# utiasSTARS/pyslam

Measured on AMD Instinct MI355X. Metric: ms/LM-iter (Jac build + J^T J + Schur solve), stereo BA @ 500k residuals, lower is better.
Workload: dtype f64

## Files before the change

### include/pyslam_hip.h

```cpp
#ifndef PYSLAM_HIP_H
#define PYSLAM_HIP_H

#include <stdint.h>

#ifdef __cplusplus
extern "C" {
#endif

typedef struct ps_problem ps_problem;

typedef struct ps_problem_desc {
    int32_t dof;
    int32_t num_poses;
    const double*  poses;
    const int32_t* pose_rid;
    int32_t num_points;
    const double*  points;
    const int32_t* point_vid;

    int64_t num_obs;
    const int32_t* obs_pose;
    const int32_t* obs_point;
    const double*  obs_uvd;
    const int32_t* obs_grp;
// ... 140 lines not shown
int ps_covariance_column(ps_problem* h, int kind, int index, int comp, double tol, int max_iters,
                         int* iters_out, double* relres_out);

#define PS_COV_DENSE_MAX_UNKNOWNS 12288
int ps_covariance_marginals(ps_problem* h, double* pose_blocks ,
                            double* point_blocks );
int ps_covariance_pose_blocks(ps_problem* h, int64_t n, const int32_t* a, const int32_t* b,
                              double* out );
int ps_covariance_cross_blocks(ps_problem* h, int64_t n, const int32_t* kind_a, const int32_t* a,
                               const int32_t* kind_b, const int32_t* b, double* out );

int ps_triangulate(ps_problem* h, int64_t n, const int32_t* vids , int refine_iters, double min_parallax_deg,
                   int write_back, double* points_out , int32_t* status_out );

int ps_get_reduced_system(ps_problem* h, int32_t* row_ptr, int32_t* col_idx,
                          double* vals, double* g);
int ps_get_landmark_factors(ps_problem* h, double* cinv , double* c );
int ps_debug_reproj_blocks(ps_problem* h, double* r , double* jpose ,
                           double* jpoint );
int ps_debug_factor_blocks(ps_problem* h, double* r, double* j1, double* j2);
int ps_debug_table_checksums(ps_problem* h, uint64_t* out, int capacity, int* count);

int ps_set_option(ps_problem* h, const char* name, double value);

int ps_set_profiling(ps_problem* h, int enabled);
int ps_get_stage_times(ps_problem* h, double* ms , int64_t* counts, int reset);

int ps_dense_normal_solve(const double* J, const double* r, int32_t m, int32_t n,
                          double* dx, double* covariance );

int ps_sparse_normal_solve(int32_t m, int32_t n, const int32_t* j_row_ptr, const int32_t* j_col, const double* j_val,
                           const int32_t* jt_row_ptr, const int32_t* jt_col, const double* jt_val,
                           const double* r, const double* rhs, double tol, int32_t max_iters,
                           double* dx, int32_t* iters_out, double* relres_out);

int ps_sparse_normal_direct(int32_t m, int32_t n, const int32_t* j_row_ptr, const int32_t* j_col, const double* j_val,
                            const int32_t* jt_row_ptr, const int32_t* jt_col, const double* jt_val,
                            const double* r, const double* rhs, int32_t refine_steps, double* dx, double* relres_out);

int ps_debug_band_inverse(const double* a, int32_t ncb, int32_t dof, int32_t bw, int32_t chunk_nodes, float* ainv_out,
                          double* elapsed_us);
int ps_debug_factor_stress(const double* a, int32_t ncb, int32_t dof, int32_t bw, int32_t mode, int32_t launches, int32_t lowprio,
                           int32_t aggressor, int32_t* n_diff, int32_t* n_pivot);

int ps_ransac_transforms(const double* pts_1, const double* pts_2, int32_t batch, int32_t n, double* T_out);
int ps_ransac_cost(const double* T, int32_t num_hyp, const double* pts_1, const double* obs_2, int32_t num_pts,
// ... 81 lines not shown
```

### pyslam_amd/_native.py

```python
import ctypes as C
import os

import numpy as np

_HERE = os.path.dirname(os.path.abspath(__file__))
LIB_PATH = os.path.join(_HERE, 'lib', 'libpyslam_hip.so')
if os.environ.get('PYSLAM_AMD_MEASURE') == '1':
    LIB_PATH = os.path.join(_HERE, 'lib', 'libpyslam_hip_measure.so')

c_i32p = C.POINTER(C.c_int32)
c_f64p = C.POINTER(C.c_double)
c_u8p = C.POINTER(C.c_uint8)
PS_NUM_STAGES = 12
STAGE_NAMES = ['landmark_pass', 'pose_pass', 'schur_pairs', 'pose_factors', 'pcg',
               'backsub', 'update', 'cost', 'iteration_total', 'cg_kernel', 'allreduce', 'pack_unpack']


class ProblemDesc(C.Structure):
    _fields_ = [
        ('dof', C.c_int32), ('num_poses', C.c_int32), ('poses', c_f64p), ('pose_rid', c_i32p),
        ('num_points', C.c_int32), ('points', c_f64p), ('point_vid', c_i32p),
        ('num_obs', C.c_int64), ('obs_pose', c_i32p), ('obs_point', c_i32p), ('obs_uvd', c_f64p),
        ('obs_grp', c_i32p),
        ('num_cams', C.c_int32), ('cams', c_f64p), ('num_stiff3', C.c_int32), ('stiff3', c_f64p),
# ... 89 lines not shown
    'ps_solve_lm': (C.c_int, [H, C.POINTER(LmOptions), C.c_double, C.c_int, c_f64p, C.c_int32, C.POINTER(C.c_int32),
                              C.POINTER(C.c_int32), C.POINTER(C.c_double), c_i32p, c_f64p, c_f64p, c_f64p]),
    'ps_gn_finish': (C.c_int, [H, C.c_int, c_f64p, c_f64p, c_f64p]),
    'ps_gn_solve_finish': (C.c_int, [H, C.c_double, C.c_int, C.c_int, c_f64p, c_f64p, c_f64p,
                                     C.POINTER(C.c_int), c_f64p]),
    'ps_set_collective': (C.c_int, [H, C.c_void_p, C.c_void_p]),
    'ps_set_segment_exchange': (C.c_int, [H, C.c_void_p, C.c_int32, C.c_int32, C.c_int64, C.c_int64, C.POINTER(C.c_int64), C.c_int64,
                                         C.POINTER(C.c_int64), C.POINTER(C.c_int64), C.POINTER(C.c_int64)]),
    'ps_shard_buffer': (C.c_int, [H, C.POINTER(C.c_void_p)]),
    'ps_gn_solve_finish_enqueue': (C.c_int, [H, C.c_double, C.c_int, C.c_int, C.c_int]),
    'ps_gn_result': (C.c_int, [H, C.POINTER(C.c_int), c_f64p, c_f64p, C.POINTER(C.c_int), c_f64p]),
    'ps_covariance_begin': (C.c_int, [H]),
    'ps_covariance_column': (C.c_int, [H, C.c_int, C.c_int, C.c_int, C.c_double, C.c_int, C.POINTER(C.c_int), c_f64p]),
    'ps_covariance_marginals': (C.c_int, [H, c_f64p, c_f64p]),
    'ps_covariance_pose_blocks': (C.c_int, [H, C.c_int64, c_i32p, c_i32p, c_f64p]),
    'ps_covariance_cross_blocks': (C.c_int, [H, C.c_int64, c_i32p, c_i32p, c_i32p, c_i32p, c_f64p]),
    'ps_triangulate': (C.c_int, [H, C.c_int64, c_i32p, C.c_int, C.c_double, C.c_int, c_f64p, c_i32p]),
    'ps_get_reduced_system': (C.c_int, [H, c_i32p, c_i32p, c_f64p, c_f64p]),
    'ps_get_landmark_factors': (C.c_int, [H, c_f64p, c_f64p]),
    'ps_debug_reproj_blocks': (C.c_int, [H, c_f64p, c_f64p, c_f64p]),
    'ps_debug_factor_blocks': (C.c_int, [H, c_f64p, c_f64p, c_f64p]),
    'ps_debug_table_checksums': (C.c_int, [H, C.POINTER(C.c_uint64), C.c_int, C.POINTER(C.c_int)]),
    'ps_set_option': (C.c_int, [H, C.c_char_p, C.c_double]),
    'ps_set_profiling': (C.c_int, [H, C.c_int]),
    'ps_get_stage_times': (C.c_int, [H, c_f64p, C.POINTER(C.c_int64), C.c_int]),
    'ps_ransac_transforms': (C.c_int, [c_f64p, c_f64p, C.c_int32, C.c_int32, c_f64p]),
    'ps_ransac_cost': (C.c_int, [c_f64p, C.c_int32, c_f64p, c_f64p, C.c_int32, c_f64p, C.c_double, c_u8p, c_i32p]),
    'ps_ransac_frame_to_frame': (C.c_int, [c_f64p, c_f64p, c_f64p, C.c_int32, c_i32p, C.c_int32, C.c_int32, c_f64p,
                                           C.c_double, c_f64p, c_i32p, c_i32p, c_i32p, c_f64p, c_u8p]),
    'ps_twoview_hypotheses': (C.c_int, [c_f64p, c_f64p, C.c_int32, c_i32p, C.c_int32, c_f64p, C.c_double, c_f64p, c_i32p, c_u8p]),
    'ps_twoview_score': (C.c_int, [c_f64p, C.c_int32, c_f64p, c_f64p, C.c_int32, c_f64p, C.c_double, c_u8p, c_i32p]),
    'ps_twoview_ransac': (C.c_int, [c_f64p, c_f64p, C.c_int32, c_i32p, C.c_int32, c_f64p, C.c_double, C.c_int32, c_f64p, c_f64p,
                                    c_u8p, c_i32p, c_f64p]),
    'ps_photometric_create': (C.c_int, [C.POINTER(PhotoDesc), C.c_void_p, C.POINTER(H)]),
    'ps_photometric_destroy': (C.c_int, [H]),
    'ps_photometric_set_pose': (C.c_int, [H, c_f64p]),
    'ps_photometric_get_pose': (C.c_int, [H, c_f64p]),
    'ps_photometric_eval_cost': (C.c_int, [H, c_f64p, C.POINTER(C.c_int64)]),
    'ps_photometric_normal_equations': (C.c_int, [H, c_f64p, c_f64p, c_f64p, C.POINTER(C.c_int64)]),
    'ps_photometric_iteration': (C.c_int, [H, C.c_int32, C.c_int32, c_f64p, c_f64p]),
    'ps_dense_create': (C.c_int, [C.c_int32, C.c_int32, C.c_int32, C.c_int32, C.c_void_p, C.POINTER(H)]),
    'ps_dense_destroy': (C.c_int, [H]),
    'ps_dense_upload': (C.c_int, [H, C.c_int32, C.c_int32, C.c_int32, C.c_int32, C.c_void_p, c_f64p]),
    'ps_dense_make_tables': (C.c_int, [H, C.c_int32, C.c_int32, c_i32p, c_f64p, C.c_double, C.c_double, C.c_double]),
    'ps_dense_track': (C.c_int, [H, C.c_int32, C.c_int32, C.c_int32, c_i32p, c_i32p, C.POINTER(SolveOptions), C.c_int32,
                                 C.c_double, c_f64p, c_f64p, c_i32p, c_f64p, C.c_int32]),
# ... 118 lines not shown
```

### pyslam_amd/csrc/ps_abi_problem.h

```cpp


const char* ps_last_error(void) { return g_err.c_str(); }

int ps_device_count(void) {
    int n = 0;
    if (hipGetDeviceCount(&n) != hipSuccess) return 0;
    return n;
}

int ps_warm_up(void) {
    static std::once_flag once;
    static int rc = 0;
    std::call_once(once, [] {
        void* p = nullptr;
        if (hipMalloc(&p, 256) != hipSuccess) { rc = fail("hipMalloc failed (no usable HIP device?)"); return; }
        hipLaunchKernelGGL(k_zero4, dim3(1), dim3(256), 0, 0, (size_t)8, (double*)p, (size_t)0, (double*)nullptr, (size_t)0,
                           (double*)nullptr, (size_t)0, (double*)nullptr);
        double hostw[4] = {0, 0, 0, 0};
        (void)hipMemsetAsync(p, 0, 256, 0);
        (void)hipMemcpyAsync((char*)p + 128, p, 64, hipMemcpyDeviceToDevice, 0);
        (void)hipMemcpyAsync(hostw, p, sizeof(hostw), hipMemcpyDeviceToHost, 0);
        if (hipDeviceSynchronize() != hipSuccess) rc = fail("the warm-up launch failed");
        hipFree(p);
        hipFuncAttributes a;
// ... 699 lines not shown
            if (rb >= 0) { cs.push_back({diag_slot[rb], base + 2 * DD, 0}); gl[rb].push_back(base + 3 * DD + D); }
            if (ra >= 0 && rb >= 0) {
                if (ra == rb) return fail("pose-pose edge connects a pose with itself");
                cs.push_back({slot_of(ra, rb), base + DD, 0});
                cs.push_back({slot_of(rb, ra), base + DD, 1});
            }
        }
        std::stable_sort(cs.begin(), cs.end(), [](const C& x, const C& y) { return x.slot < y.slot; });
        std::vector<int32_t> eslots, eptr, ediag, gptr(nr + 1, 0), gitems;
        std::vector<int2> eitems(cs.size());
        for (size_t k = 0; k < cs.size(); ++k) {
            eitems[k] = make_int2(cs[k].off, cs[k].tr);
            if (k == 0 || cs[k].slot != cs[k - 1].slot) { eslots.push_back(cs[k].slot); eptr.push_back((int32_t)k); }
        }
        eptr.push_back((int32_t)cs.size());
        for (int32_t s : eslots) {
            const int row = (int)(std::upper_bound(row_ptr.begin(), row_ptr.end(), s) - row_ptr.begin()) - 1;
            ediag.push_back(col_idx[s] == row ? 1 : 0);
        }
        for (int r = 0; r < nr; ++r) { gptr[r + 1] = gptr[r] + (int32_t)gl[r].size(); gitems.insert(gitems.end(), gl[r].begin(), gl[r].end()); }
        h->nes = (int)eslots.size();
        if (h->upload(&h->eslots, eslots) || h->upload(&h->eptr, eptr) || h->upload(&h->eslot_diag, ediag) ||
            h->upload(&h->eitems, eitems) || h->upload(&h->gptr, gptr) || h->upload(&h->gitems, gitems)) return -1;
    }

    lap("factor lists");
    const size_t nvec = (size_t)nr * D;
    h->npartA = std::max(1, nr);
    h->npartB = std::max(1, cdiv(nr, D == 6 ? PS_PCG_BR(6) : PS_PCG_BR(3)));
    h->hist_cap = 4098;
    if (h->alloc(&h->x, nvec) || h->alloc(&h->r, nvec) || h->alloc(&h->z, nvec) || h->alloc(&h->p0, nvec) ||
        h->alloc(&h->p1, nvec) || h->alloc(&h->q, nvec) || h->alloc(&h->Minv, (size_t)nr * DD) ||
        h->alloc(&h->rz_part, h->npartB) || h->alloc(&h->rr_part, h->npartB) || h->alloc(&h->pq_part, h->npartA) ||
        h->alloc(&h->hist, 2 * (size_t)h->hist_cap)) return -1;
    {
        std::vector<int32_t> brow_of(nnzb), ident(nnzb);
        for (int r = 0; r < nr; ++r) for (int b = row_ptr[r]; b < row_ptr[r + 1]; ++b) brow_of[b] = r;
        for (int b = 0; b < nnzb; ++b) ident[b] = b;
        if (h->upload(&h->brow_of, brow_of) || h->upload(&h->ident_slot, ident)) return -1;
        if (h->alloc(&h->Linv, (size_t)nr * DD)) return -1;
    }
    if (h->zero(h->x, nvec * sizeof(double)) || h->zero(h->p0, nvec * sizeof(double)) || h->zero(h->p1, nvec * sizeof(double))) return -1;

    lap("pcg workspace");
    h->ncost_obs = N > 0 ? std::min(2048, cdiv(N, 256)) : 0;
    h->ncost_fac = F > 0 ? std::min(1024, cdiv(F, 256)) : 0;
// ... 42 lines not shown
    char* whost = (char*)h->words_host;
    h->h_scalars = (double*)(whost + 0);      h->h_scalars_dev = (double*)(wdev + 0);
    h->h_status = (int32_t*)(whost + 256);    h->h_status_dev = (int32_t*)(wdev + 256);
    h->h_seq = (long long*)(whost + 512);     h->h_seq_dev = (long long*)(wdev + 512);
    h->h_shard = (double*)(whost + 768);      h->h_shard_dev = (double*)(wdev + 768);
    h->h_setup = (long long*)(whost + 1024);  h->h_setup_dev = (long long*)(wdev + 1024);
    h->h_ldi_fro = (double*)(whost + 1280);   h->h_ldi_fro_dev = (double*)(wdev + 1280);
    h->h_early = (long long*)(whost + 1536);  h->h_early_dev = (long long*)(wdev + 1536);
    h->h_lmfail = (long long*)(whost + 1792); h->h_lmfail_dev = (long long*)(wdev + 1792);
    h->h_mo_hist = (double*)(whost + 2048);   h->h_mo_hist_dev = (double*)(wdev + 2048);
    if (h->alloc(&h->arrivals, 2)) return -1;
    if (h->zero(h->arrivals, 2 * sizeof(int32_t))) return -1;
    if (h->arena_close()) return -1;
    HIP_OK(hipStreamSynchronize(h->stream));
    if (nr >= 16 && nr * D > h->direct_max && h->pcg_variant == 1 && !ps_env("PS_LAZY_COARSE")) {
        if (build_coarse(h)) return -1;
        HIP_OK(hipStreamSynchronize(h->stream));
        lap("two-level structures");
    }
    if (ldi_eligible(h) && h->ldi_direct_ok && h->N == 0 && h->F > 0 && !h->ldi_stream &&
        !ps_pool().take(ps_pool().side_streams, &h->ldi_stream))
        HIP_OK(hipStreamCreateWithFlags(&h->ldi_stream, hipStreamNonBlocking));
    lap("scalars + final sync");
    guard.ok = true;
    *out = h;
    return 0;
}

int ps_problem_create(const ps_problem_desc* d_in, void* stream, ps_problem** out) {
    return problem_create(d_in, nullptr, stream, out);
}

int ps_problem_create_hybrid(const ps_problem_desc* d_in, const ps_host_rows_desc* rows, void* stream, ps_problem** out) {
    if (!rows) return fail("null argument");
    return problem_create(d_in, rows, stream, out);
}

int ps_set_host_rows(ps_problem* h, const double* rows, int64_t num, double cost) {
    if (!h) return fail("null argument");
    if (!h->hybrid) return fail("ps_set_host_rows: the handle has no host rows (ps_problem_create_hybrid)");
    if (num != h->FH) return fail("ps_set_host_rows: row count differs from the create call's");
    if (num > 0 && !rows) return fail("null argument");
    const size_t FROW = 3 * (size_t)h->D * h->D + 2 * (size_t)h->D;
    if (num > 0) {
        HIP_OK(hipMemcpyAsync(h->fscratch + (size_t)h->F * FROW, rows, (size_t)num * FROW * sizeof(double), hipMemcpyHostToDevice, h->stream));
        HIP_OK(hipStreamSynchronize(h->stream));
// ... 7 lines not shown
```

### pyslam_amd/csrc/ps_abi_solver.h

```cpp

int ps_get_info(ps_problem* h, ps_problem_info* info) {
    if (!h || !info) return fail("null argument");
    info->dof = h->D; info->num_poses = h->P; info->num_reduced = h->nr; info->num_points = h->L;
    info->num_var_points = h->nv; info->num_obs = h->N; info->num_edges = h->F; info->num_priors = 0;
    info->reduced_nnzb = h->nnzb; info->num_pairs = h->npairs;
    info->reduce_count = ((long)h->nnzb + h->nr) / 2 * h->D * h->D + (long)h->nr * h->D + 3;
    info->device_bytes = (int64_t)h->dev_bytes;
    info->cg_restarts = h->cg_fallbacks;
    info->cg_kernel_launches = h->cg_kernel_launches;
    info->ldi_solves = h->ldi_solves; info->ldi_fallbacks = h->ldi_fallbacks; info->ldi_seeds = h->ldi_seeds;
    info->xcg_fused_solves = h->xf_solves; info->xcg_fused_fallbacks = h->xf_fallbacks;
    info->cg_persist_solves = h->cp_launches; info->cg_persist_failures = h->cp_failures;
    info->cg_persist_refused = h->cp_refused; info->persist_cus = h->persist_cus;
    info->persist_cus_needed = h->cp_ok ? h->cp_cus_needed : (h->xp_ok ? h->xp_cus_needed : 0);
    info->landmark_passes_taken_over = h->prelm_used;
    return 0;
}

int ps_eval_cost(ps_problem* h, int include_all_constant, double* cost) {
    if (!h || !cost) return fail("null argument");
    if (include_all_constant && h->fuse_cost == 1 && lm_cost_possible(h)) { if (lm_cost_pass(h, h->lin_lambda, SC_COST)) return -1; }
    else if (cost_pass(h, include_all_constant, SC_COST)) return -1;
    if (read_scalars(h)) return -1;
    *cost = h->h_scalars[SC_COST];
// ... 5 lines not shown
    if (!h) return fail("null argument");
    h->last_cost = h->prev_cost = -1.0;
    return linearize(h, lambda);
}

static int ensure_shard_pack(ps_problem* h) {
    if (h->shard_pack) return 0;
    const int nr = h->nr, DD = h->D * h->D;
    std::vector<int32_t> up, upT;
    for (int r = 0; r < nr; ++r)
        for (int b = h->h_row_ptr[r]; b < h->h_row_ptr[r + 1]; ++b) {
            const int c = h->h_col_idx[b];
            if (c < r) continue;
            up.push_back(b);
            const int32_t* lo = h->h_col_idx.data() + h->h_row_ptr[c];
            const int32_t* hi = h->h_col_idx.data() + h->h_row_ptr[c + 1];
            const int32_t* it = std::lower_bound(lo, hi, r);
            if (it == hi || *it != r) return fail("reduced block pattern is not symmetric");
            upT.push_back((int32_t)(it - h->h_col_idx.data()));
        }
    h->nup = (long)up.size();
    h->pack_count = h->nup * DD + (long)nr * h->D + 2 + 1;
    if (h->upload(&h->up_slot, up) || h->upload(&h->upT_slot, upT) || h->alloc(&h->shard_pack, (size_t)h->pack_count)) return -1;
    return 0;
}

int ps_reduce_buffer(ps_problem* h, void** dev_ptr, int64_t* count) {
    if (!h || !dev_ptr || !count) return fail("null argument");
    if (ensure_shard_pack(h)) return -1;
    *dev_ptr = h->shard_pack; *count = h->pack_count;
    return 0;
}

int ps_shard_pack(ps_problem* h) {
    if (!h) return fail("null argument");
    if (ensure_shard_pack(h)) return -1;
    const long ntail = (long)h->nr * h->D + 2;
    const int nb = (int)std::min<long>(4096, cdiv(h->pack_count, 256));
    if (h->D == 6) hipLaunchKernelGGL(k_shard_pack<6>, dim3(nb), dim3(256), 0, h->stream, h->nup, h->up_slot, h->S, ntail, h->g, h->status, h->shard_pack);
    else hipLaunchKernelGGL(k_shard_pack<3>, dim3(nb), dim3(256), 0, h->stream, h->nup, h->up_slot, h->S, ntail, h->g, h->status, h->shard_pack);
    return 0;
}

int ps_shard_unpack(ps_problem* h) {
    if (!h) return fail("null argument");
    h->prelin_valid = h->prelm_valid = false;
// ... 199 lines not shown
    {
        StageTimer tpk(h, PS_ST_PACK);
        if (h->D == 6) hipLaunchKernelGGL(k_seg_pack<6>, dim3(nb1), dim3(256), 0, h->stream, h->nup, h->up_slot, h->S, ntail, h->g, h->status, T, h->seg_nmine, h->seg_mine, h->seg_in, h->seg_maxlen);
        else hipLaunchKernelGGL(k_seg_pack<3>, dim3(nb1), dim3(256), 0, h->stream, h->nup, h->up_slot, h->S, ntail, h->g, h->status, T, h->seg_nmine, h->seg_mine, h->seg_in, h->seg_maxlen);
    }
    {
        StageTimer tar(h, PS_ST_ALLREDUCE);
        if (h->seg_allgather(h->seg_in, h->seg_all, (size_t)h->seg_maxlen, NCCL_F64, h->nccl_comm, h->stream))
            return fail("ncclAllGather of the reduced system's segments failed");
    }
    {
        StageTimer tpk(h, PS_ST_PACK);
        if (h->D == 6) hipLaunchKernelGGL(k_seg_sum<6>, dim3(nb2), dim3(256), 0, h->stream, h->seg_ndst, h->seg_dst, h->seg_src_ptr, h->seg_src_off, h->seg_all, T, h->seg_world, h->seg_maxlen, h->nup, h->up_slot, h->upT_slot, h->S, ntail, h->g, h->status);
        else hipLaunchKernelGGL(k_seg_sum<3>, dim3(nb2), dim3(256), 0, h->stream, h->seg_ndst, h->seg_dst, h->seg_src_ptr, h->seg_src_off, h->seg_all, T, h->seg_world, h->seg_maxlen, h->nup, h->up_slot, h->upT_slot, h->S, ntail, h->g, h->status);
    }
    return 0;
}

int ps_set_collective(ps_problem* h, void* nccl_all_reduce_fn, void* nccl_comm) {
    if (!h) return fail("null argument");
    if (h->hybrid && nccl_comm) return fail("a hybrid handle (host rows) is not landmark-sharded");
    h->nccl_allreduce = (ps_problem::allreduce_fn)nccl_all_reduce_fn;
    h->nccl_comm = nccl_comm;
    return 0;
}

int ps_shard_buffer(ps_problem* h, void** dev_ptr) {
    if (!h || !dev_ptr) return fail("null argument");
    *dev_ptr = h->shard_buf;
    return 0;
}

int ps_gn_solve_finish_enqueue(ps_problem* h, double pcg_tol, int pcg_max_iters, int linesearch, int first) {
    if (!h) return fail("null argument");
    if (h->nr == 0 || h->pcg_variant != 1) return fail("ps_gn_solve_finish_enqueue needs the fused CG and a reduced system");
    pcg_tol = resolve_pcg_tol(h, pcg_tol);
    if (first && z_of_last_linearize(h, "ps_gn_solve_finish_enqueue")) return -1;
    h->shard_out = true;
    h->no_repeat = !(h->nccl_allreduce && h->nccl_comm);
    struct Reset { ps_problem* h; ~Reset() { h->shard_out = false; h->no_repeat = false; } } reset{h};
    if (first) {
        HIP_OK(hipMemsetAsync(h->scalars + SC_DXP2, 0, sizeof(double), h->stream));
        if (!h->coarse_built && build_coarse(h)) return -1;
        if (!(h->nccl_allreduce && h->nccl_comm) && h->xf_skip == 0) h->xf_skip = 1;
        if (h->cg_explicit) { if (h->D == 6 ? xcg_setup<6>(h, pcg_max_iters, true) : xcg_setup<3>(h, pcg_max_iters, true)) return -1; }
        else if (h->D == 6 ? cg_fused_setup<6>(h, pcg_max_iters, true) : cg_fused_setup<3>(h, pcg_max_iters, true)) return -1;
// ... 547 lines not shown
    else if (n == "ldi_cap") { if (value < 1 || value > 64) return fail("ldi_cap out of range (1 .. 64)"); h->ldi_cap = (int)value; }
    else if (n == "ldi_cost_tol") { if (!(value >= 0)) return fail("ldi_cost_tol must be >= 0"); h->ldi_cost_tol = value; }
    else if (n == "ldi_refresh_its") { if (value < 0 || value > 64) return fail("ldi_refresh_its out of range (0 .. 64)"); h->ldi_refresh_its = (int)value; }
    else if (n == "ldi_direct") { h->ldi_direct_ok = value != 0.0; h->ldi_direct = value > 0.0; }
    else if (n == "direct_fused") h->direct_fused = value != 0.0;
    else if (n == "ldi_seed_lag") { if (value < 1 || value > 16) return fail("ldi_seed_lag out of range (1 .. 16)"); h->ldi_seed_lag = (int)value; }
    else if (n == "ldi_seed_steps") { if (value < 1 || value > 40) return fail("ldi_seed_steps out of range (1 .. 40)"); h->ldi_seed_steps = (int)value; }
    else if (n == "coarse_refresh_every") { if (value < 1 || value > 16) return fail("coarse_refresh_every must be 1..16"); h->xcg_refresh_every = (int)value; }
    else if (n == "coarse_lag_x") { h->lagx = value != 0.0; h->lci_next = -1; h->side_todo = false; }
    else if (n == "cg_lds") h->cg_lds = value != 0.0;
    else if (n == "cg_persist") h->cg_persist = value != 0.0;
    else if (n == "xcg_persist") h->xcg_persist = value != 0.0;
    else if (n == "cg_persist_spin") { if (value < 0 || value > 1e7) return fail("cg_persist_spin out of range"); h->cp_spin = (unsigned)value; }
    else if (n == "cg_explicit") { h->explicit_ok = value != 0.0; h->coarse_built = false; }
    else if (n == "big_chol") h->big_chol = value != 0.0;
    else if (n == "fused_motion_only") h->mo_fused = value != 0.0;
    else if (n == "direct_max_unknowns") { if (value < 0 || value > 90) return fail("direct_max_unknowns must be 0..90"); h->direct_max = (int)value; }
    else if (n == "coarse_basis") { h->coarse_basis = value != 0.0; h->lci_next = -1; h->side_todo = false; }
    else if (n == "profile_every") { if (value < 1) return fail("profile_every must be >= 1"); h->prof_every = (int)value; }
    else if (n == "cg_margin") { if (value < 0 || value > 64) return fail("cg_margin out of range"); h->cg_margin = (int)value; }
    else if (n == "cg_split_min_rows") { h->cg_split_min_rows = (int)value; h->coarse_built = false; }
    else if (n == "cg_explicit_min_rows") { h->cg_explicit_min_rows = (int)value; h->coarse_built = false; }
    else if (n == "pcg_chunk") { if (value < 1 || value > 4096) return fail("pcg_chunk out of range"); h->pcg_chunk = (int)value; }
    else return fail("unknown option: " + n);
    return 0;
}

int ps_reset_solver_state(ps_problem* h) {
    if (!h) return fail("null argument");
    h->prelin_valid = h->prelm_valid = false;
    if (!h->solver_touched) {
        h->last_cost = h->prev_cost = h->snap_cost = -1.0;
        h->solve_horizon = -1;
        return 0;
    }
    h->solver_touched = false;
    HIP_OK(hipStreamSynchronize(h->stream));
    if (h->side) HIP_OK(hipStreamSynchronize(h->side));
    if (h->ldi_stream) HIP_OK(hipStreamSynchronize(h->ldi_stream));
    drain_timers(h);
    h->lci_next = -1; h->lci_cur = 0;
    h->side_todo = false; h->side_ready = false; h->side_pending = false; h->acdone_pending = false;
    h->xcg_side_todo = false; h->xcg_lag_count = 0; h->xcg_held = 0;
    h->xcg_its_ref = 0; h->xcg_good_held = 0; h->xcg_ref_pending = false;
    h->xcg_tag[0] = h->xcg_tag[1] = -1.0; h->xcg_tag_lambda[0] = h->xcg_tag_lambda[1] = 0.0;
    h->xcg_setup_cost = -1.0; h->xcg_setup_lambda = 0.0;
    h->mc_active = false; h->last_setup_lagx = false; h->xf_skip = 0;
// ... 67 lines not shown
```

### pyslam_amd/csrc/ps_core.hip

```cpp
#include <hip/hip_runtime.h>

#include <algorithm>
#include <array>
#include <map>
#include <atomic>
#include <chrono>
#include <thread>
#include <climits>
#include <cmath>
#include <cstdio>
#include <cstring>
#include <memory>
#include <mutex>
#include <string>
#include <vector>

#include "pyslam_hip.h"
#include "ps_kernels.h"
#include "ps_ransac.h"
#include "ps_k_twoview.h"
#include "ps_photo.h"
#include "ps_k_dense.h"
#include "ps_k_feat.h"
#include "ps_sparse.h"
// ... 135 lines not shown
    LObs* pobs = nullptr;
    PItem* pitems = nullptr;
    int npitems = 0;
    int32_t* pitem_ptr = nullptr;
    double* ppartial = nullptr;
    int2* pairs = nullptr;
    int npair_items = 0, pair_per_xcd = 0;
    PairItem* pair_xitems = nullptr;
    int schur_tiles = 1, ncomb = 0;
    bool has_diag_tasks = false;
    double* Spart = nullptr;
    PairItem* comb_items = nullptr;
    int32_t* comb_tasks = nullptr;
    FactorGroup* fgroups = nullptr;
    int32_t *f_i = nullptr, *f_j = nullptr, *f_grp = nullptr;
    double *f_Tinv = nullptr, *fscratch = nullptr;
    int32_t *eslots = nullptr, *eptr = nullptr, *eslot_diag = nullptr, *gptr = nullptr, *gitems = nullptr;
    int2* eitems = nullptr;
    int nes = 0;
    int32_t *row_ptr = nullptr, *col_idx = nullptr, *diag_slot = nullptr;
    double* red = nullptr;
    long red_count = 0;
    double *S = nullptr, *g = nullptr, *red_cost = nullptr;
    std::vector<int32_t> h_row_ptr, h_col_idx;
    std::vector<int32_t> h_vid_of_slot;
    double *x = nullptr, *r = nullptr, *z = nullptr, *p0 = nullptr, *p1 = nullptr, *q = nullptr, *Minv = nullptr;
    double *rz_part = nullptr, *rr_part = nullptr, *pq_part = nullptr, *hist = nullptr;
    int npartA = 0, npartB = 0, hist_cap = 0, last_pcg_iters = 0;
    int pcg_variant = 1;
    int pcg_chunk = 8;
    double *Linv = nullptr, *cg_r[2] = {}, *cg_w[2] = {}, *cg_s[2] = {}, *cg_gd[2] = {}, *cg_xh = nullptr;
    int32_t* brow_of = nullptr;
    double* cg_p = nullptr;
    double* Saug = nullptr;
    int32_t* ident_slot = nullptr;
    int coarse_req = -1;
    int G = 0, ncb = 0, nc = 0, nr_aug = 0, nnzb_aug = 0;
    size_t cg_cap = 0, saug_cap = 0;
    int32_t *pnode = nullptr, *slo = nullptr, *shi = nullptr, *run_lo = nullptr, *run_hi = nullptr,
            *arow_ptr = nullptr, *acol_idx = nullptr, *aug_slot = nullptr, *fine_nnz = nullptr;
    double *pw0 = nullptr, *pw1 = nullptr, *SZ = nullptr, *Ac = nullptr, *tvec = nullptr, *chol_scratch = nullptr;
    int coarse_basis = 1;
    double *Bmat = nullptr, *bgv = nullptr, *SB = nullptr, *BSZ = nullptr;
    double *Bmat2[2] = {}, *X2[2] = {}, *Mpart = nullptr;
    bool lagx_ok = false;
    int lagx = 1;
// ... 318 lines not shown
    int arena_close() {
        arena_open = false;
        if (arena_poisoned) arena_used = PS_ARENA_BYTES;
        if (arena_used) HIP_OK(hipMemcpyAsync(arena_dev, arena_host, arena_used, hipMemcpyHostToDevice, stream));
        return 0;
    }
    void arena_release() {
        PsPool& pool = ps_pool();
        if (arena_dev && !pool.give(pool.dev_arenas, (void*)arena_dev)) hipFree(arena_dev);
        if (arena_host && !pool.give(pool.host_arenas, (void*)arena_host)) hipHostFree(arena_host);
        if (words_host && !pool.give(pool.host_words, words_host)) hipHostFree(words_host);
        arena_dev = arena_host = nullptr; words_host = nullptr;
    }
};

inline void cov_release(ps_problem* h) {
    if (!h->cov_buf) return;
    hipStreamSynchronize(h->stream);
    hipFree(h->cov_buf);
    h->cov_buf = nullptr;
    h->cov_sigma_epoch = -1;
}

#include "ps_host_cg.h"
#include "ps_host_ldi.h"
#include "ps_host_iteration.h"
#include "ps_host_build.h"

extern "C" {

#include "ps_abi_problem.h"
#include "ps_abi_solver.h"
#include "ps_abi_cov.h"
#include "ps_abi_triang.h"
#include "ps_abi_small.h"
#include "ps_abi_twoview.h"
#include "ps_abi_dense.h"
#include "ps_abi_feat.h"

}
```

### pyslam_amd/csrc/ps_host_cg.h

```cpp

namespace {

struct StageTimer {
    ps_problem* h;
    int stage;
    hipEvent_t a = nullptr, b = nullptr;
    int slot = -1;
    StageTimer(ps_problem* h_, int st, int level = 2) : h(h_), stage(st) {
        if (h->profiling < level) return;
        if (h->profiling == 1 && h->prof_every > 1 &&
            h->prof_tick % h->prof_every != (st == PS_ST_CG_KERNEL ? h->prof_every / 2 : 0)) return;
        if (h->ev_used + 2 > h->ev_pool.size()) {
            for (int i = 0; i < 64; ++i) { hipEvent_t e; hipEventCreate(&e); h->ev_pool.push_back(e); }
        }
        slot = (int)h->ev_used;
        a = h->ev_pool[h->ev_used++];
        b = h->ev_pool[h->ev_used++];
        hipEventRecord(a, h->stream);
    }
    void stop() {
        if (!a) return;
        hipEventRecord(b, h->stream);
        h->pending.push_back({stage, slot});
        a = nullptr;
// ... 848 lines not shown
    if (iters_out) *iters_out = total_its;
    if (relres_out) *relres_out = rel * reduced;
    h->last_pcg_iters = total_its;
    return rc;
}

int linearize(ps_problem* h, double lambda, bool allow_prelm) {
    h->solver_touched = true;
    h->prelin_valid = false;
    const bool lm_done = allow_prelm && h->prelm_valid && h->prelm_lambda == lambda && h->nv > 0;
    h->prelm_valid = false;
    h->lin_lmfail_tag = lm_done ? h->prelm_tag : 0;
    if (lm_done) ++h->prelm_used;
    h->lin_lambda = lambda;
    h->params_moved_since_lin = false; h->z_foreign = false;
    ++h->prof_tick;
    h->cov_ready = false;
    cov_release(h);
    h->status_clean = false;
    if (h->ldi_sread_pending) {
        HIP_OK(hipStreamWaitEvent(h->stream, h->ev_ldi_sread, 0));
        h->ldi_sread_pending = false;
    }
    HIP_OK(hipMemsetAsync(h->red, 0, h->red_count * sizeof(double) + ST_NWORDS * sizeof(int32_t), h->stream));
    if (h->nv > 0 && !lm_done) {
        StageTimer t(h, PS_ST_LANDMARK);
        const ObsWide wl{h->sidx_l, h->stiff_tab};
#define PS_LM_LAUNCH(W) hipLaunchKernelGGL(k_landmark_pass<W>, dim3(cdiv(h->nv, 256 / PS_LM_GROUP)), dim3(256), 0, h->stream, h->nv, h->lm_ptr, \
                           h->lm_point, h->lobs, h->poses, h->points, h->pose_rid, h->ogroups, lambda, h->Z,                       \
                           h->Cinv, h->cvec, h->status, h->lm_ablate, wl)
#define PS_LMP_LAUNCH(W) hipLaunchKernelGGL((k_landmark_pass_packed<W, false>), dim3(cdiv(h->lmw_nwaves, 4)), dim3(256), 0, h->stream, h->lmw_nwaves, \
                           h->lmw_first, h->lm_ptr, h->lm_point, h->lobs, h->poses, h->points, h->pose_rid, h->ogroups, lambda, h->Z,      \
                           h->Cinv, h->cvec, h->status, wl, (const int32_t*)nullptr, (double*)nullptr, (long long*)nullptr, 0LL)
        if (h->lm_packed && h->lmw_nwaves > 0 && !h->lm_ablate) { if (h->wide_obs) PS_LMP_LAUNCH(true); else PS_LMP_LAUNCH(false); }
        else if (h->wide_obs) PS_LM_LAUNCH(true); else PS_LM_LAUNCH(false);
#undef PS_LMP_LAUNCH
#undef PS_LM_LAUNCH
    }
    bool fin_in_combine = false, fin_in_pairs = false;
    static const bool schur_split_env = ps_env("PS_SCHUR_SPLIT") != nullptr;
    if (h->npitems > 0) {
        StageTimer t(h, PS_ST_POSE);
        const ObsWide wp{h->sidx_p, h->stiff_tab};
        const int per_xcd = h->pose_xcd ? cdiv(h->npitems, 8) : 0;
        const int nblk = per_xcd ? 8 * per_xcd : h->npitems;
        if (h->wide_obs)
            hipLaunchKernelGGL(k_pose_pass<true>, dim3(nblk), dim3(256), 0, h->stream, h->pitems, h->pobs,
                               h->poses, h->points, h->ogroups, h->Cinv, h->cvec, h->ppartial, lambda != 0.0 ? 1 : 0, wp, h->npitems, per_xcd);
        else
            hipLaunchKernelGGL(k_pose_pass<false>, dim3(nblk), dim3(256), 0, h->stream, h->pitems, h->pobs,
                               h->poses, h->points, h->ogroups, h->Cinv, h->cvec, h->ppartial, lambda != 0.0 ? 1 : 0, wp, h->npitems, per_xcd);
        fin_in_combine = h->Spart && h->npair_items > 0 && !h->has_diag_tasks && h->D == 6;
        fin_in_pairs = !h->Spart && h->schur_pipeline && h->npair_items > 0 && !h->has_diag_tasks && h->D == 6 && !schur_split_env;
        if (!fin_in_combine && !fin_in_pairs)
            hipLaunchKernelGGL(k_pose_finalize, dim3(h->nr), dim3(64), 0, h->stream, h->nr, h->pitem_ptr,
                               h->ppartial, h->diag_slot, lambda, h->S, h->g);
    }
    if (h->npair_items > 0) {
        StageTimer t(h, PS_ST_SCHUR, 1);
        const bool split2 = schur_split_env;
        const int halfp = split2 ? (h->pair_per_xcd / 2 + 3) / 4 * 4 : h->pair_per_xcd;
        static const int lds_pad = ps_env("PS_SCHUR_LDS_PAD") ? atoi(ps_env("PS_SCHUR_LDS_PAD")) : 0;
        auto launch_pairs = [&](int nblk, int lds, int from, int to) {
            if (!h->schur_pipeline)
                hipLaunchKernelGGL(k_schur_pairs, dim3(nblk), dim3(256), lds, h->stream, h->pair_per_xcd, h->pair_xitems, h->pairs,
                                   h->Z, h->S, h->Spart, h->schur_ablate, from, to);
            else {
#ifdef PS_MEASURE
                auto k = h->schur_ablate == 0 ? k_schur_pairs_db<0> : h->schur_ablate == 1 ? k_schur_pairs_db<1> :
                         h->schur_ablate == 2 ? k_schur_pairs_db<2> : h->schur_ablate == 3 ? k_schur_pairs_db<3> :
                         h->schur_ablate == 4 ? k_schur_pairs_db<4> : k_schur_pairs_db<5>;
#else
                auto k = k_schur_pairs_db<0>;
#endif
// ... 219 lines not shown
```

### pyslam_amd/csrc/ps_k_linearize.h

```cpp
#pragma once

#define PS_LM_GROUP 16

PS_DEV double group16_sum(double v) {
    v = dpp_shift_add<0x111, 0xf, 0xf>(v);
    v = dpp_shift_add<0x112, 0xf, 0xf>(v);
    v = dpp_shift_add<0x114, 0xf, 0xe>(v);
    v = dpp_shift_add<0x118, 0xf, 0xc>(v);
    return __shfl(v, (int)(threadIdx.x & 63) | 15, 64);
}

#define PS_ZROW 16

PS_DEV void lm_emit_m(const ReprojEval& ev, double M00, double M10, double M11, double M20, double M21,
                      double M22, double* __restrict__ m) {
#pragma unroll
    for (int a = 0; a < 3; ++a) {
        const double w0 = ev.Jp[a] * ev.Jl[0] + ev.Jp[6 + a] * ev.Jl[3] + ev.Jp[12 + a] * ev.Jl[6];
        const double w1 = ev.Jp[a] * ev.Jl[1] + ev.Jp[6 + a] * ev.Jl[4] + ev.Jp[12 + a] * ev.Jl[7];
        const double w2 = ev.Jp[a] * ev.Jl[2] + ev.Jp[6 + a] * ev.Jl[5] + ev.Jp[12 + a] * ev.Jl[8];
        m[3 * a] = w0 * M00;
        m[3 * a + 1] = w0 * M10 + w1 * M11;
        m[3 * a + 2] = w0 * M20 + w1 * M21 + w2 * M22;
    }
// ... 152 lines not shown
    acc[17] += y * F[2][2] - z * F[1][2];
    acc[18] += z * F[0][1] - x * F[2][1];
    acc[19] += z * F[0][2] - x * F[2][2];
    acc[20] += x * F[1][2] - y * F[0][2];
}

#define PS_NPOSE_ACC 33
#ifndef PS_POSE_TRANSPOSE
#define PS_POSE_TRANSPOSE 1
#endif
typedef const __attribute__((address_space(1))) void* ps_gptr_t;
typedef __attribute__((address_space(3))) void* ps_lptr_t;

#ifndef PS_POSE_WAVES
#define PS_POSE_WAVES 3
#endif
template <bool WIDE>
__global__ __launch_bounds__(256) __attribute__((amdgpu_waves_per_eu(PS_POSE_WAVES, 8))) void k_pose_pass(
    const PItem* __restrict__ items,
    const LObs* __restrict__ pobs ,
    const double* __restrict__ poses, const double* __restrict__ points,
    const ObsGroup* __restrict__ groups, const double* __restrict__ Cinv,
    const double* __restrict__ cvec, double* __restrict__ partial, int want_diag ,
    ObsWide wide, int nitems, int per_xcd )
{
    __shared__ double red[4][PS_NPOSE_ACC];
#if PS_POSE_TRANSPOSE
    __shared__ double tr[4][64 * 17];
#endif
    const int item = per_xcd > 0 ? (int)(blockIdx.x & 7) * per_xcd + (int)(blockIdx.x >> 3) : (int)blockIdx.x;
    if (item >= nitems) return;
    const PItem it = items[item];
    const int w = threadIdx.x >> 6, lane = threadIdx.x & 63;
    const Se3 T = se3_load(poses + 12 * (size_t)it.pad);
    double acc[PS_NPOSE_ACC];
#pragma unroll
    for (int k = 0; k < PS_NPOSE_ACC; ++k) acc[k] = 0.0;
    for (int i = it.start + threadIdx.x; i < it.end; i += 256) {
        const LObs o = pobs[i];
        const int v = PS_POSE_OF(o) - 1;
        const double pw[3] = {points[3 * (size_t)o.point], points[3 * (size_t)o.point + 1], points[3 * (size_t)o.point + 2]};
        double m[6] = {0, 0, 0, 0, 0, 0}, c0 = 0.0, c1 = 0.0, c2 = 0.0;
        if (v >= 0) {
            const double* ci = Cinv + 6 * (size_t)v;
#pragma unroll
            for (int k = 0; k < 6; ++k) m[k] = ci[k];
            c0 = cvec[3 * (size_t)v]; c1 = cvec[3 * (size_t)v + 1]; c2 = cvec[3 * (size_t)v + 2];
        }
        ReprojEval ev;
        reproj_eval_obs<true, true, WIDE>(T, pw, &o.u, groups, PS_GRP_OF(o), wide, i, ev);
        double G[6], t3[3];
        {
// ... 355 lines not shown
```

### pyslam_amd/device.py

```python
import ctypes as C

import numpy as np

from pyslam_amd import _native as nat


COVARIANCE_MARGINALS_LIMIT = 12288


def _solve_options(o, opt, linesearch=None):
    o.max_iters, o.allow_nondecreasing_steps = int(opt.max_iters), int(bool(opt.allow_nondecreasing_steps))
    o.max_nondecreasing_steps = int(opt.max_nondecreasing_steps)
    o.linesearch = int(bool(opt.linesearch_max_iters > 0 if linesearch is None else linesearch))
    o.min_update_norm, o.min_cost = float(opt.min_update_norm), float(opt.min_cost)
    o.min_cost_decrease, o.lm_lambda = float(opt.min_cost_decrease), float(getattr(opt, 'lm_lambda', 0.))
    return o


class DeviceProblem:
    def __init__(self, lp, stream=None, extra_pairs=None):
        lib = nat.require_gpu()
        self._lib = lib
        self.lp = lp
        self.dof = lp.dof
# ... 363 lines not shown
    def get_info(self):
        info = nat.ProblemInfo()
        nat.check(self._lib.ps_get_info(self._h, C.byref(info)))
        return {k: getattr(info, k) for k, _ in nat.ProblemInfo._fields_}

    def cg_restarts(self):
        info = nat.ProblemInfo()
        nat.check(self._lib.ps_get_info(self._h, C.byref(info)))
        return int(info.cg_restarts)

    def cg_kernel_launches(self):
        info = nat.ProblemInfo()
        nat.check(self._lib.ps_get_info(self._h, C.byref(info)))
        return int(info.cg_kernel_launches)

    def cg_persist_counts(self):
        info = nat.ProblemInfo()
        nat.check(self._lib.ps_get_info(self._h, C.byref(info)))
        return int(info.cg_persist_solves), int(info.cg_persist_failures)

    def set_option(self, name, value):
        nat.check(self._lib.ps_set_option(self._h, name.encode(), float(value)))

    def set_profiling(self, level=2):
        nat.check(self._lib.ps_set_profiling(self._h, int(level)))

    def stage_times(self, reset=False):
        ms = (C.c_double * nat.PS_NUM_STAGES)()
        cnt = (C.c_int64 * nat.PS_NUM_STAGES)()
        nat.check(self._lib.ps_get_stage_times(self._h, ms, cnt, int(reset)))
        return {n: (ms[i], cnt[i]) for i, n in enumerate(nat.STAGE_NAMES)}


def dense_normal_solve(J, r, want_covariance=False):
    lib = nat.require_gpu()
    J = np.ascontiguousarray(J, dtype=np.float64)
    r = np.ascontiguousarray(r, dtype=np.float64).reshape(-1)
    m, n = J.shape
    dx = np.zeros(n)
    cov = np.zeros((n, n)) if want_covariance else None
    nat.check(lib.ps_dense_normal_solve(nat.f64p(J), nat.f64p(r), m, n, nat.f64p(dx), nat.f64p(cov)))
    return (dx, cov) if want_covariance else dx


def band_inverse(A, ncb, dof, bw, chunk_nodes=0):
    lib = nat.require_gpu()
# ... 267 lines not shown
```

Before: 0.3064.

## Replace full reduction-buffer memset with targeted slot zeroing fused into pose pass

Instead of memsetting the whole Schur/gradient reduction buffer every linearization, a host-side analysis finds the block slots that are not fully overwritten by a single writer. Extra blocks are appended to the pose-pass kernel launch to zero only those slots plus the gradient/status tail. This removes a large memset pass over S each iteration and folds the remaining clearing into an existing launch. It relies on the single-writer analysis being correct, is gated off for sharded, extra-pair or non-pipelined configurations, and adds a get_option read-back API.

Result: faster. 0.3031 (median of 6 runs) (-1.1%).

```diff
diff --git a/include/pyslam_hip.h b/include/pyslam_hip.h
--- a/include/pyslam_hip.h
+++ b/include/pyslam_hip.h
@@ -186,6 +186,7 @@
 int ps_debug_table_checksums(ps_problem* h, uint64_t* out, int capacity, int* count);
 
 int ps_set_option(ps_problem* h, const char* name, double value);
+int ps_get_option(ps_problem* h, const char* name, double* value);
 
 int ps_set_profiling(ps_problem* h, int enabled);
 int ps_get_stage_times(ps_problem* h, double* ms , int64_t* counts, int reset);
diff --git a/pyslam_amd/_native.py b/pyslam_amd/_native.py
--- a/pyslam_amd/_native.py
+++ b/pyslam_amd/_native.py
@@ -135,6 +135,7 @@
     'ps_debug_factor_blocks': (C.c_int, [H, c_f64p, c_f64p, c_f64p]),
     'ps_debug_table_checksums': (C.c_int, [H, C.POINTER(C.c_uint64), C.c_int, C.POINTER(C.c_int)]),
     'ps_set_option': (C.c_int, [H, C.c_char_p, C.c_double]),
+    'ps_get_option': (C.c_int, [H, C.c_char_p, c_f64p]),
     'ps_set_profiling': (C.c_int, [H, C.c_int]),
     'ps_get_stage_times': (C.c_int, [H, c_f64p, C.POINTER(C.c_int64), C.c_int]),
     'ps_ransac_transforms': (C.c_int, [c_f64p, c_f64p, C.c_int32, C.c_int32, c_f64p]),
diff --git a/pyslam_amd/csrc/ps_abi_problem.h b/pyslam_amd/csrc/ps_abi_problem.h
--- a/pyslam_amd/csrc/ps_abi_problem.h
+++ b/pyslam_amd/csrc/ps_abi_problem.h
@@ -745,6 +745,20 @@
         h->nes = (int)eslots.size();
         if (h->upload(&h->eslots, eslots) || h->upload(&h->eptr, eptr) || h->upload(&h->eslot_diag, ediag) ||
             h->upload(&h->eitems, eitems) || h->upload(&h->gptr, gptr) || h->upload(&h->gitems, gitems)) return -1;
+        if (D == 6 && ntiles == 1 && nnzb > 0) {
+            std::vector<uint8_t> writers((size_t)nnzb, 0);
+            for (const PairItem& it : pitm) {
+                if (it.slot >= 0 && writers[it.slot] < 2) ++writers[it.slot];
+                if (it.slotT >= 0 && it.slotT != it.slot && writers[it.slotT] < 2) ++writers[it.slotT];
+            }
+            for (int32_t s : eslots) if (s >= 0) writers[s] = 2;
+            for (int r = 0; r < nr; ++r) writers[diag_slot[r]] = 2;
+            std::vector<int32_t> zl;
+            for (int b = 0; b < nnzb; ++b) if (writers[b] != 1) zl.push_back(b);
+            h->nzero_slots = (int)zl.size();
+            if (!zl.empty() && h->upload(&h->zero_slots, zl)) return -1;
+        }
+        h->has_extra_pairs = d->num_extra_pairs > 0;
     }
 
     lap("factor lists");
@@ -833,6 +847,7 @@
         !ps_pool().take(ps_pool().side_streams, &h->ldi_stream))
         HIP_OK(hipStreamCreateWithFlags(&h->ldi_stream, hipStreamNonBlocking));
     lap("scalars + final sync");
+    relook_launch_gates(h);
     guard.ok = true;
     *out = h;
     return 0;
diff --git a/pyslam_amd/csrc/ps_abi_solver.h b/pyslam_amd/csrc/ps_abi_solver.h
--- a/pyslam_amd/csrc/ps_abi_solver.h
+++ b/pyslam_amd/csrc/ps_abi_solver.h
@@ -51,6 +51,7 @@
     h->nup = (long)up.size();
     h->pack_count = h->nup * DD + (long)nr * h->D + 2 + 1;
     if (h->upload(&h->up_slot, up) || h->upload(&h->upT_slot, upT) || h->alloc(&h->shard_pack, (size_t)h->pack_count)) return -1;
+    relook_launch_gates(h);
     return 0;
 }
 
@@ -296,6 +297,7 @@
     if (h->hybrid && nccl_comm) return fail("a hybrid handle (host rows) is not landmark-sharded");
     h->nccl_allreduce = (ps_problem::allreduce_fn)nccl_all_reduce_fn;
     h->nccl_comm = nccl_comm;
+    relook_launch_gates(h);
     return 0;
 }
 
@@ -889,7 +891,19 @@
     else if (n == "cg_split_min_rows") { h->cg_split_min_rows = (int)value; h->coarse_built = false; }
     else if (n == "cg_explicit_min_rows") { h->cg_explicit_min_rows = (int)value; h->coarse_built = false; }
     else if (n == "pcg_chunk") { if (value < 1 || value > 4096) return fail("pcg_chunk out of range"); h->pcg_chunk = (int)value; }
+    else if (n == "lin_zero_list") h->lin_zero_list = value != 0.0;
     else return fail("unknown option: " + n);
+    relook_launch_gates(h);
+    return 0;
+}
+
+int ps_get_option(ps_problem* h, const char* name, double* value) {
+    if (!h || !name || !value) return fail("null argument");
+    const std::string n(name);
+    if (n == "lin_zero_list") *value = h->lin_zero_gate ? 1.0 : 0.0;
+    else if (n == "lin_fills") *value = (double)h->lin_fills;
+    else if (n == "lin_zero_launches") *value = (double)h->lin_zero_launches;
+    else return fail("ps_get_option: no read-back for option: " + n);
     return 0;
 }
 
diff --git a/pyslam_amd/csrc/ps_core.hip b/pyslam_amd/csrc/ps_core.hip
--- a/pyslam_amd/csrc/ps_core.hip
+++ b/pyslam_amd/csrc/ps_core.hip
@@ -181,6 +181,12 @@
     double* red = nullptr;
     long red_count = 0;
     double *S = nullptr, *g = nullptr, *red_cost = nullptr;
+    int32_t* zero_slots = nullptr;
+    int nzero_slots = 0;
+    bool has_extra_pairs = false;
+    int lin_zero_list = 1;
+    bool lin_zero_gate = false;
+    long lin_fills = 0, lin_zero_launches = 0;
     std::vector<int32_t> h_row_ptr, h_col_idx;
     std::vector<int32_t> h_vid_of_slot;
     double *x = nullptr, *r = nullptr, *z = nullptr, *p0 = nullptr, *p1 = nullptr, *q = nullptr, *Minv = nullptr;
@@ -545,6 +551,11 @@
     h->cov_sigma_epoch = -1;
 }
 
+inline void relook_launch_gates(ps_problem* h) {
+    const bool shard = (h->nccl_allreduce && h->nccl_comm) || h->seg_allgather || h->shard_pack || h->has_extra_pairs;
+    h->lin_zero_gate = h->lin_zero_list && h->zero_slots && !h->Spart && h->schur_pipeline && h->npitems > 0 && h->D == 6 && !shard;
+}
+
 #include "ps_host_cg.h"
 #include "ps_host_ldi.h"
 #include "ps_host_iteration.h"
diff --git a/pyslam_amd/csrc/ps_host_cg.h b/pyslam_amd/csrc/ps_host_cg.h
--- a/pyslam_amd/csrc/ps_host_cg.h
+++ b/pyslam_amd/csrc/ps_host_cg.h
@@ -894,8 +894,16 @@
         HIP_OK(hipStreamWaitEvent(h->stream, h->ev_ldi_sread, 0));
         h->ldi_sread_pending = false;
     }
-    HIP_OK(hipMemsetAsync(h->red, 0, h->red_count * sizeof(double) + ST_NWORDS * sizeof(int32_t), h->stream));
-    if (h->nv > 0 && !lm_done) {
+    const bool zero_by_list = h->lin_zero_gate;
+    const bool lm_here = h->nv > 0 && !lm_done;
+    if (!zero_by_list) {
+        HIP_OK(hipMemsetAsync(h->red, 0, h->red_count * sizeof(double) + ST_NWORDS * sizeof(int32_t), h->stream));
+        ++h->lin_fills;
+    } else {
+        if (lm_here) HIP_OK(hipMemsetAsync(h->status, 0, ST_NWORDS * sizeof(int32_t), h->stream));
+        ++h->lin_zero_launches;
+    }
+    if (lm_here) {
         StageTimer t(h, PS_ST_LANDMARK);
         const ObsWide wl{h->sidx_l, h->stiff_tab};
 #define PS_LM_LAUNCH(W) hipLaunchKernelGGL(k_landmark_pass<W>, dim3(cdiv(h->nv, 256 / PS_LM_GROUP)), dim3(256), 0, h->stream, h->nv, h->lm_ptr, \
@@ -916,12 +924,18 @@
         const ObsWide wp{h->sidx_p, h->stiff_tab};
         const int per_xcd = h->pose_xcd ? cdiv(h->npitems, 8) : 0;
         const int nblk = per_xcd ? 8 * per_xcd : h->npitems;
+        static_assert(ST_NWORDS % 2 == 0, "the status words are cleared as doubles");
+        const int ntail = zero_by_list ? h->nr * 6 + 2 + (lm_here ? 0 : ST_NWORDS / 2) : 0;
+        const int nzs = zero_by_list ? h->nzero_slots : 0;
+        const int nzblk = zero_by_list ? cdiv((long)nzs * 36 + ntail, 256) : 0;
         if (h->wide_obs)
-            hipLaunchKernelGGL(k_pose_pass<true>, dim3(nblk), dim3(256), 0, h->stream, h->pitems, h->pobs,
-                               h->poses, h->points, h->ogroups, h->Cinv, h->cvec, h->ppartial, lambda != 0.0 ? 1 : 0, wp, h->npitems, per_xcd);
+            hipLaunchKernelGGL(k_pose_pass<true>, dim3(nblk + nzblk), dim3(256), 0, h->stream, h->pitems, h->pobs,
+                               h->poses, h->points, h->ogroups, h->Cinv, h->cvec, h->ppartial, lambda != 0.0 ? 1 : 0, wp, h->npitems, per_xcd,
+                               nblk, (const int32_t*)h->zero_slots, nzs, h->S, h->g, ntail);
         else
-            hipLaunchKernelGGL(k_pose_pass<false>, dim3(nblk), dim3(256), 0, h->stream, h->pitems, h->pobs,
-                               h->poses, h->points, h->ogroups, h->Cinv, h->cvec, h->ppartial, lambda != 0.0 ? 1 : 0, wp, h->npitems, per_xcd);
+            hipLaunchKernelGGL(k_pose_pass<false>, dim3(nblk + nzblk), dim3(256), 0, h->stream, h->pitems, h->pobs,
+                               h->poses, h->points, h->ogroups, h->Cinv, h->cvec, h->ppartial, lambda != 0.0 ? 1 : 0, wp, h->npitems, per_xcd,
+                               nblk, (const int32_t*)h->zero_slots, nzs, h->S, h->g, ntail);
         fin_in_combine = h->Spart && h->npair_items > 0 && !h->has_diag_tasks && h->D == 6;
         fin_in_pairs = !h->Spart && h->schur_pipeline && h->npair_items > 0 && !h->has_diag_tasks && h->D == 6 && !schur_split_env;
         if (!fin_in_combine && !fin_in_pairs)
diff --git a/pyslam_amd/csrc/ps_k_linearize.h b/pyslam_amd/csrc/ps_k_linearize.h
--- a/pyslam_amd/csrc/ps_k_linearize.h
+++ b/pyslam_amd/csrc/ps_k_linearize.h
@@ -198,12 +198,19 @@
     const double* __restrict__ poses, const double* __restrict__ points,
     const ObsGroup* __restrict__ groups, const double* __restrict__ Cinv,
     const double* __restrict__ cvec, double* __restrict__ partial, int want_diag ,
-    ObsWide wide, int nitems, int per_xcd )
+    ObsWide wide, int nitems, int per_xcd ,
+    int zero_first, const int32_t* __restrict__ zero_slots, int nzero_slots, double* __restrict__ S, double* __restrict__ ztail, int ntail)
 {
     __shared__ double red[4][PS_NPOSE_ACC];
 #if PS_POSE_TRANSPOSE
     __shared__ double tr[4][64 * 17];
 #endif
+    if ((int)blockIdx.x >= zero_first) {
+        const int e = ((int)blockIdx.x - zero_first) * 256 + (int)threadIdx.x, ns = 36 * nzero_slots;
+        if (e < ns) { const int k = e / 36; S[(size_t)zero_slots[k] * 36 + (e - 36 * k)] = 0.0; }
+        else if (e - ns < ntail) ztail[e - ns] = 0.0;
+        return;
+    }
     const int item = per_xcd > 0 ? (int)(blockIdx.x & 7) * per_xcd + (int)(blockIdx.x >> 3) : (int)blockIdx.x;
     if (item >= nitems) return;
     const PItem it = items[item];
diff --git a/pyslam_amd/device.py b/pyslam_amd/device.py
--- a/pyslam_amd/device.py
+++ b/pyslam_amd/device.py
@@ -409,6 +409,11 @@
     def set_option(self, name, value):
         nat.check(self._lib.ps_set_option(self._h, name.encode(), float(value)))
 
+    def get_option(self, name):
+        v = C.c_double()
+        nat.check(self._lib.ps_get_option(self._h, name.encode(), C.byref(v)))
+        return v.value
+
     def set_profiling(self, level=2):
         nat.check(self._lib.ps_set_profiling(self._h, int(level)))
 
```
